# Hongyang-Du/VideoGPA

Measured on AMD Instinct MI355X. Metric: DPO preference-pair steps/sec, CogVideoX-5B 49f@480x720, higher is better.
Workload: dtype bf16; 1 GPU; BASELINE configs[1]: CogVideoX-5B T2V full (42 blocks, D=3072, 48x64 heads), 49f x 480x720 -> paired latents [1,2,13,16,60,90], S=17776 tokens, 42 blocks, LoRA r=64 on to_q/to_k/to_v/to_out.0, 1 pair/GPU/step, optimizer step every step; random-init weights; layers=42, pairs_per_gpu=1, parallelism=dp1

## Files before the change

### videogpa_amd/csrc/lora.hip

```cpp
#include "attn_w1.h"

#ifndef LORA_DOWN_DMA
#define LORA_DOWN_DMA 1
#endif
#ifndef LORA_DOWN_DMA_NCB
#define LORA_DOWN_DMA_NCB 2
#endif
#ifndef LORA_DOWN_NS
#define LORA_DOWN_NS 4
#endif
#ifndef LORA_GRAD_WGS
#define LORA_GRAD_WGS 768
#endif

#include <cstdlib>

__device__ __forceinline__ void tile_load_zfill(const bf16_t* base, int64_t ld, int64_t row0, int64_t nrows, int col0, int ncols,
                                                u32x4_t (&r)[2]) {
#pragma unroll
    for (int j = 0; j < 2; ++j) {
        const int c = threadIdx.x + 256 * j;
        const int64_t row = row0 + (c >> 3);
        const int col = col0 + (c & 7) * 8;
        u32x4_t z = {0u, 0u, 0u, 0u};
        r[j] = (row < nrows && col < ncols) ? *reinterpret_cast<const u32x4_t*>(base + row * ld + col) : z;
    }
}

template <int NCB>
__global__ __launch_bounds__(256) void lora_down_kernel(const bf16_t* __restrict__ X, int64_t ldx, const bf16_t* __restrict__ A,
                                                          bf16_t* __restrict__ T, int64_t ldt, int64_t M, int K, int R) {
    extern __shared__ __attribute__((aligned(16))) bf16_t smem[];
    constexpr int RP = 32 * NCB;
    constexpr int NACC = (NCB + 1) / 2;
    constexpr int BUF = (64 + RP) * PITCH;
    const int lane = threadIdx.x & 63, wave = threadIdx.x >> 6, hi = lane >> 5;
    const int rb = wave & 1, cg = wave >> 1;
    const int64_t row0 = (int64_t)blockIdx.x * 64;

    f32x16_t acc[NACC];
#pragma unroll
    for (int a = 0; a < NACC; ++a)
#pragma unroll
        for (int i = 0; i < 16; ++i) acc[a][i] = 0.f;

    u32x4_t xr[2], ar[NCB];
    auto load = [&](int k0) {
        tile_load_zfill(X, ldx, row0, M, k0, K, xr);
#pragma unroll
        for (int j = 0; j < NCB; ++j) {
            const int c = threadIdx.x + 256 * j;
            const int row = c >> 3;
            u32x4_t z = {0u, 0u, 0u, 0u};
            ar[j] = (row < R) ? *reinterpret_cast<const u32x4_t*>(A + (int64_t)row * K + k0 + (c & 7) * 8) : z;
        }
    };
    auto store = [&](int buf) {
        bf16_t* xl = smem + buf * BUF;
        bf16_t* al = xl + 64 * PITCH;
        tile_store(xl, xr);
#pragma unroll
        for (int j = 0; j < NCB; ++j) {
            const int c = threadIdx.x + 256 * j;
            *reinterpret_cast<u32x4_t*>(al + (c >> 3) * PITCH + (c & 7) * 8) = ar[j];
        }
    };
    const int nk = K / 64;
    load(0);
    store(0);
    __syncthreads();
    for (int t = 0; t < nk; ++t) {
        const bf16_t* xl = smem + (t & 1) * BUF;
        const bf16_t* al = xl + 64 * PITCH;
        if (t + 1 < nk) load((t + 1) * 64);
#pragma unroll
        for (int ks = 0; ks < 4; ++ks) {
            const bf16x8_t xf = frag_row(xl, rb * 32, ks, lane);
#pragma unroll
            for (int a = 0; a < NACC; ++a) {
                const int cb = cg + 2 * a;
                if (cb < NCB) acc[a] = mfma32(frag_row(al, cb * 32, ks, lane), xf, acc[a]);
            }
        }
        if (t + 1 < nk) store((t + 1) & 1);
        __syncthreads();
    }
    const int64_t m = row0 + rb * 32 + (lane & 31);
    if (m < M) {
#pragma unroll
        for (int a = 0; a < NACC; ++a) {
            const int cb = cg + 2 * a;
            if (cb < NCB) {
#pragma unroll
                for (int g = 0; g < 4; ++g) {
                    const int n = cb * 32 + 8 * g + 4 * hi;
                    if (n + 3 < R || n < R) {
                        if (n + 3 < R) {
                            u32x2_t w;
                            w[0] = pack_bf16x2(acc[a][4 * g], acc[a][4 * g + 1]);
                            w[1] = pack_bf16x2(acc[a][4 * g + 2], acc[a][4 * g + 3]);
                            *reinterpret_cast<u32x2_t*>(T + m * ldt + n) = w;
                        } else {
                            for (int i = 0; i < 4; ++i)
                                if (n + i < R) T[m * ldt + n + i] = f32_to_bf16(acc[a][4 * g + i]);
                        }
                    }
                }
            }
        }
    }
}

template <int N>
__device__ __forceinline__ void lora_wait_vm() { asm volatile("s_waitcnt vmcnt(%0) lgkmcnt(0)" ::"n"(N) : "memory"); }

template <int NCB, int NS>
__global__ __launch_bounds__(256) void lora_down_dma_kernel(const bf16_t* __restrict__ X, int64_t ldx, const bf16_t* __restrict__ A, bf16_t* __restrict__ T,
                                                              int64_t ldt, int64_t M, int K, int R) {
    constexpr int RP = 32 * NCB;
    constexpr int NACC = (NCB + 1) / 2;
    constexpr int STAGE = 8192 + RP * 128;
    constexpr int PW = 2 + NCB;
    __shared__ __attribute__((aligned(1024))) uint8_t lds[NS * STAGE];
    const int lane = threadIdx.x & 63, hi = lane >> 5;
    const int wave = __builtin_amdgcn_readfirstlane((int)threadIdx.x >> 6);
    const int rb = wave & 1, cg = wave >> 1;
    const int64_t row0 = (int64_t)blockIdx.x * 64;
    const int64_t rows = (M - row0) < 64 ? (M - row0) : 64;

    const W1Rsrc xrs = w1_rsrc(X + row0 * ldx, (uint32_t)(((rows - 1) * ldx + K) * 2));
    const W1Rsrc ars = w1_rsrc(A, (uint32_t)((int64_t)R * K * 2));
    uint32_t xo[2], ao[NCB];
#pragma unroll
    for (int i = 0; i < 2; ++i) {
        const uint32_t row = 8u * (uint32_t)(wave * 2 + i) + (uint32_t)(lane >> 3);
        xo[i] = (uint32_t)((row * (uint64_t)ldx + (((uint32_t)(lane & 7) ^ w1_swz(row)) * 8u)) * 2u);
    }
#pragma unroll
    for (int i = 0; i < NCB; ++i) {
        const uint32_t row = 8u * (uint32_t)(wave * NCB + i) + (uint32_t)(lane >> 3);
        ao[i] = (row * (uint32_t)K + (((uint32_t)(lane & 7) ^ w1_swz(row)) * 8u)) * 2u;
    }
    const uint32_t lds0 = (uint32_t)(uintptr_t)(__attribute__((address_space(3))) uint8_t*)lds;
    const uint32_t xdst = __builtin_amdgcn_readfirstlane(lds0 + (uint32_t)wave * 2048u);
    const uint32_t adst = __builtin_amdgcn_readfirstlane(lds0 + 8192u + (uint32_t)wave * (uint32_t)NCB * 1024u);
    auto issue = [&](int slot) {
        const uint32_t so = (uint32_t)slot * (uint32_t)STAGE;
#pragma unroll
        for (int i = 0; i < 2; ++i) { w1_dma(xdst + so + 1024u * i, xrs, xo[i], 0u); xo[i] += 128u; }
#pragma unroll
        for (int i = 0; i < NCB; ++i) { w1_dma(adst + so + 1024u * i, ars, ao[i], 0u); ao[i] += 128u; }
    };
    f32x16_t acc[NACC];
#pragma unroll
    for (int a = 0; a < NACC; ++a)
#pragma unroll
        for (int i = 0; i < 16; ++i) acc[a][i] = 0.f;
    const W1Lane la = w1_lane_offsets(lane);
    const int nk = K / 64;
#pragma unroll
    for (int t = 0; t < NS - 1; ++t) issue(t);
    for (int t = 0; t < nk; ++t) {
        lora_wait_vm<PW * (NS - 2)>();
        __syncthreads();
        issue((t + NS - 1) % NS);
        const uint32_t xb = (uint32_t)(t % NS) * (uint32_t)STAGE, ab = xb + 8192u;
#pragma unroll
        for (int ks = 0; ks < 4; ++ks) {
            const bf16x8_t xf = w1_frag_row(lds, xb, la, rb, ks);
#pragma unroll
            for (int a = 0; a < NACC; ++a) {
                const int cb = cg + 2 * a;
                if (cb < NCB) acc[a] = mfma32(w1_frag_row(lds, ab, la, cb, ks), xf, acc[a]);
            }
        }
    }
    lora_wait_vm<0>();
    const int64_t m = row0 + rb * 32 + (lane & 31);
    if (m < M) {
#pragma unroll
        for (int a = 0; a < NACC; ++a) {
            const int cb = cg + 2 * a;
            if (cb < NCB) {
#pragma unroll
                for (int g = 0; g < 4; ++g) {
                    const int n = cb * 32 + 8 * g + 4 * hi;
                    if (n + 3 < R) {
                        u32x2_t w;
                        w[0] = pack_bf16x2(acc[a][4 * g], acc[a][4 * g + 1]);
                        w[1] = pack_bf16x2(acc[a][4 * g + 2], acc[a][4 * g + 3]);
                        *reinterpret_cast<u32x2_t*>(T + m * ldt + n) = w;
                    } else {
                        for (int i = 0; i < 4; ++i)
                            if (n + i < R) T[m * ldt + n + i] = f32_to_bf16(acc[a][4 * g + i]);
                    }
                }
            }
        }
    }
}

#ifndef UP_COLS
#define UP_COLS 128
#endif
#define UP_PITCH (UP_COLS + 4)
template <int KS>
__global__ __launch_bounds__(256) void lora_up_add_kernel(bf16_t* __restrict__ Y, int64_t ldy, const bf16_t* __restrict__ T, int64_t ldt,
                                                            const bf16_t* __restrict__ Bw, int64_t ldb, float s, int64_t M, int N,
                                                            int accumulate) {
    __shared__ __attribute__((aligned(16))) float tile[64 * UP_PITCH];
    const int lane = threadIdx.x & 63, wave = threadIdx.x >> 6, hi = lane >> 5;
    const int64_t m0 = (int64_t)blockIdx.x * 64;
    const int n0 = blockIdx.y * UP_COLS;
    const int rb = wave & 1, cg = wave >> 1;
    int64_t mr = m0 + rb * 32 + (lane & 31);
    mr = mr < M ? mr : M - 1;
    bf16x8_t tf[KS];
#pragma unroll
    for (int ks = 0; ks < KS; ++ks) tf[ks] = *reinterpret_cast<const bf16x8_t*>(T + mr * ldt + ks * 16 + hi * 8);
#pragma unroll
    for (int cbi = 0; cbi < UP_COLS / 64; ++cbi) {
        const int nl = cg * (UP_COLS / 2) + cbi * 32;
        int nrow = n0 + nl + (lane & 31);
        nrow = nrow < N ? nrow : N - 1;
        f32x16_t acc;
#pragma unroll
        for (int i = 0; i < 16; ++i) acc[i] = 0.f;
        const bf16_t* bp = Bw + (int64_t)nrow * ldb + hi * 8;
#pragma unroll
        for (int ks = 0; ks < KS; ++ks) acc = mfma32(*reinterpret_cast<const bf16x8_t*>(bp + ks * 16), tf[ks], acc);
        float* tp = tile + (rb * 32 + (lane & 31)) * UP_PITCH + nl + 4 * hi;
#pragma unroll
        for (int g = 0; g < 4; ++g) {
            f32x4_t v = {s * acc[4 * g], s * acc[4 * g + 1], s * acc[4 * g + 2], s * acc[4 * g + 3]};
            *reinterpret_cast<f32x4_t*>(tp + 8 * g) = v;
        }
    }
    __syncthreads();
#pragma unroll
    for (int j = 0; j < UP_COLS / 32; ++j) {
        const int c = threadIdx.x + 256 * j;
        const int row = c / (UP_COLS / 8), col = (c % (UP_COLS / 8)) * 8;
        const int64_t m = m0 + row;
        if (m < M && n0 + col < N) {
            const float* tp = tile + row * UP_PITCH + col;
            const f32x4_t a0 = *reinterpret_cast<const f32x4_t*>(tp), a1 = *reinterpret_cast<const f32x4_t*>(tp + 4);
            float o[8] = {a0[0], a0[1], a0[2], a0[3], a1[0], a1[1], a1[2], a1[3]};
            bf16_t* yp = Y + m * ldy + n0 + col;
            if (accumulate) {
                float y[8];
                unpack8(*reinterpret_cast<const u32x4_t*>(yp), y);
#pragma unroll
                for (int i = 0; i < 8; ++i) o[i] += y[i];
            }
            *reinterpret_cast<u32x4_t*>(yp) = pack8(o);
        }
    }
}

__global__ __launch_bounds__(256) void lora_grad_kernel(const bf16_t* __restrict__ U, int64_t ldu, const bf16_t* __restrict__ V, int64_t ldv,
                                                          float* __restrict__ G, int64_t ldg, float s, int64_t M, int P, int Q,
                                                          int64_t rows_per_split, int n_qt, float* __restrict__ part) {
    __shared__ __attribute__((aligned(16))) bf16_t lds[4 * TILE_ELEMS];
    const int lane = threadIdx.x & 63, wave = threadIdx.x >> 6, hi = lane >> 5;
    const int pb = wave & 1, qb = wave >> 1;
    const int p0 = (blockIdx.x / n_qt) * 64, q0 = (blockIdx.x % n_qt) * 64;
    const int64_t mbeg = (int64_t)blockIdx.y * rows_per_split;
    int64_t mend = mbeg + rows_per_split;
    mend = mend < M ? mend : M;
    if (mbeg >= mend) return;
    f32x16_t acc;
#pragma unroll
    for (int i = 0; i < 16; ++i) acc[i] = 0.f;
    u32x4_t ur[2], vr[2];
    const int nt = (int)((mend - mbeg + 63) / 64);
    tile_load_zfill(U, ldu, mbeg, mend, p0, P, ur);
    tile_load_zfill(V, ldv, mbeg, mend, q0, Q, vr);
    tile_store(lds, ur);
    tile_store(lds + 2 * TILE_ELEMS, vr);
    __syncthreads();
    for (int t = 0; t < nt; ++t) {
        const bf16_t* ul = lds + (t & 1) * TILE_ELEMS;
        const bf16_t* vl = lds + (2 + (t & 1)) * TILE_ELEMS;
        if (t + 1 < nt) {
            tile_load_zfill(U, ldu, mbeg + (int64_t)(t + 1) * 64, mend, p0, P, ur);
            tile_load_zfill(V, ldv, mbeg + (int64_t)(t + 1) * 64, mend, q0, Q, vr);
        }
#pragma unroll
        for (int kc = 0; kc < 4; ++kc) acc = mfma32(frag_tr(ul, 16 * kc, pb * 32, lane), frag_tr(vl, 16 * kc, qb * 32, lane), acc);
        if (t + 1 < nt) {
            tile_store(lds + ((t + 1) & 1) * TILE_ELEMS, ur);
            tile_store(lds + (2 + ((t + 1) & 1)) * TILE_ELEMS, vr);
        }
        __syncthreads();
    }
    const int q = q0 + qb * 32 + (lane & 31);
    if (q < Q) {
        float* slab = part ? part + (int64_t)blockIdx.y * P * Q : nullptr;
#pragma unroll
        for (int r = 0; r < 16; ++r) {
            const int p = p0 + pb * 32 + acc_row(r, hi);
            if (p < P) {
                if (slab) slab[(int64_t)p * Q + q] = acc[r];
                else atomicAdd(&G[(int64_t)p * ldg + q], s * acc[r]);
            }
        }
    }
}

__global__ __launch_bounds__(256) void lora_grad_merge_kernel(const float* __restrict__ part, int nsplit, float* __restrict__ G, int64_t ldg, float s,
                                                                int P, int Q) {
    const int64_t i = (int64_t)blockIdx.x * 256 + threadIdx.x;
    if (i >= (int64_t)P * Q) return;
    float a = 0.f;
    for (int c = 0; c < nsplit; ++c) a += part[(int64_t)c * P * Q + i];
    G[(i / Q) * ldg + (i % Q)] = s * a;
}

__global__ __launch_bounds__(256) void lora_ext_refresh_kernel(const float* __restrict__ A, const float* __restrict__ B, float s, int r, int K, int Dn,
                                                                 bf16_t* __restrict__ a_cat, bf16_t* __restrict__ wt_tail, int64_t ld_wt,
                                                                 bf16_t* __restrict__ w_tail, int64_t ld_w, bf16_t* __restrict__ sbt) {
    const int64_t idx = (int64_t)blockIdx.x * 256 + threadIdx.x;
    const int64_t na = (int64_t)r * K;
    if (idx < na) {
        const int rr = (int)(idx / K), kk = (int)(idx % K);
        const bf16_t a = f32_to_bf16(A[idx]);
        a_cat[idx] = a;
        wt_tail[(int64_t)kk * ld_wt + rr] = a;
    } else if (idx < na + (int64_t)Dn * r) {
        const int64_t e = idx - na;
        const int n = (int)(e / r), rr = (int)(e % r);
        const bf16_t v = f32_to_bf16(bf16_to_f32(f32_to_bf16(B[e])) * s);
        w_tail[(int64_t)n * ld_w + rr] = v;
        sbt[(int64_t)rr * Dn + n] = v;
    }
}

static inline bool a16(const void* p) { return ((uintptr_t)p & 15) == 0; }
static inline bool a8(const void* p) { return ((uintptr_t)p & 7) == 0; }

extern "C" {

int32_t vgpa_lora_down(const void* X, int64_t ldx, const void* A, void* T, int64_t ldt, int64_t M, int64_t K, int64_t R, hipStream_t stream) {
    if (!X || !A || !T || M <= 0 || K <= 0 || K % 64 != 0 || R <= 0 || R > 256 || ldx % 8 || ldt % 8 || ldx < K || ldt < R || !a16(X) || !a16(A) || !a8(T))
        return VGPA_ERR_INVALID;
    if (M > ((int64_t)1 << 31) * 32) return VGPA_ERR_INVALID;
    const int ncb = (int)((R + 31) / 32);
    const dim3 grid((unsigned)((M + 63) / 64));
    constexpr bool dma_off = LORA_DOWN_DMA == 0;
    constexpr int dma_max_ncb = LORA_DOWN_DMA_NCB;
    if (!dma_off && ncb <= dma_max_ncb && (uint64_t)64 * (uint64_t)ldx * 2 + (uint64_t)K * 2 + 1024 < (1ull << 32) && ((uint64_t)R + 8) * (uint64_t)K * 2 + 1024 < (1ull << 32)) {
#define LDD(N, S) VGPA_LAUNCH((lora_down_dma_kernel<N, S>), grid, dim3(256), 0, stream, (const bf16_t*)X, ldx, (const bf16_t*)A, (bf16_t*)T, ldt, M, (int)K, (int)R)
        constexpr int ns = LORA_DOWN_NS;
        switch (ncb * 10 + ns) {
            case 14: LDD(1, 4); break; case 24: LDD(2, 4); break;
            case 13: LDD(1, 3); break; case 23: LDD(2, 3); break;
            case 63: LDD(6, 3); break; case 64: LDD(6, 4); break;
            default: return VGPA_ERR_INVALID;
        }
#undef LDD
        VGPA_CHECK_LAUNCH();
        return VGPA_OK;
    }
    const size_t shmem = (size_t)2 * (64 + 32 * ncb) * PITCH * sizeof(bf16_t);
#define LD(N)                                                                                                                      \
    if (hipFuncSetAttribute((const void*)lora_down_kernel<N>, hipFuncAttributeMaxDynamicSharedMemorySize, (int)shmem) != hipSuccess) \
        return VGPA_ERR_LAUNCH;                                                                                                    \
    VGPA_LAUNCH((lora_down_kernel<N>), grid, dim3(256), shmem, stream, (const bf16_t*)X, ldx, (const bf16_t*)A, (bf16_t*)T, ldt, M, (int)K, (int)R)
    switch (ncb) {
        case 1: LD(1); break; case 2: LD(2); break; case 3: LD(3); break; case 4: LD(4); break;
        case 5: LD(5); break; case 6: LD(6); break; case 7: LD(7); break; case 8: LD(8); break;
        default: return VGPA_ERR_INVALID;
    }
#undef LD
    VGPA_CHECK_LAUNCH();
    return VGPA_OK;
}

int32_t vgpa_lora_up_add(void* Y, int64_t ldy, const void* T, int64_t ldt, const void* Bw, int64_t ldb, float s, int64_t M, int64_t N,
                         int64_t rp, int32_t accumulate, hipStream_t stream) {
    if (!Y || !T || !Bw || M <= 0 || N <= 0 || N % 8 != 0 || ldy % 8 || ldt % 8 || ldb % 8 || !a16(T) || !a16(Bw) || !a16(Y))
        return VGPA_ERR_INVALID;
    if (ldy < N || ldt < rp || ldb < rp) return VGPA_ERR_INVALID;
    const dim3 grid((unsigned)((M + 63) / 64), (unsigned)((N + UP_COLS - 1) / UP_COLS));
#define UP(KS) VGPA_LAUNCH((lora_up_add_kernel<KS>), grid, dim3(256), 0, stream, (bf16_t*)Y, ldy, (const bf16_t*)T, ldt, (const bf16_t*)Bw, ldb, s, M, (int)N, (int)accumulate)
    switch (rp) {
        case 16: UP(1); break; case 32: UP(2); break; case 48: UP(3); break; case 64: UP(4); break;
        case 96: UP(6); break; case 128: UP(8); break; case 192: UP(12); break;
        default: return VGPA_ERR_INVALID;
    }
#undef UP
    VGPA_CHECK_LAUNCH();
    return VGPA_OK;
}

static void lora_grad_plan(int64_t M, int64_t P, int64_t Q, int* n_pt, int* n_qt, int64_t* rows, int64_t* splits) {
    *n_pt = (int)((P + 63) / 64);
    *n_qt = (int)((Q + 63) / 64);
    constexpr int64_t target = LORA_GRAD_WGS;
    int64_t sp = target / ((int64_t)*n_pt * *n_qt);
    if (sp < 1) sp = 1;
    const int64_t max_splits = (M + 255) / 256;
    if (sp > max_splits) sp = max_splits;
    int64_t r = (M + sp - 1) / sp;
    r = (r + 63) / 64 * 64;
    *rows = r;
    *splits = (M + r - 1) / r;
}

size_t vgpa_lora_grad_workspace_bytes(int64_t M, int64_t P, int64_t Q) {
    if (M <= 0 || P <= 0 || Q <= 0) return 0;
    int n_pt, n_qt;
    int64_t rows, splits;
    lora_grad_plan(M, P, Q, &n_pt, &n_qt, &rows, &splits);
    return (size_t)splits * (size_t)P * (size_t)Q * sizeof(float);
}
int32_t vgpa_lora_grad_ws(const void* U, int64_t ldu, const void* V, int64_t ldv, float* G, int64_t ldg, float s, int64_t M, int64_t P,
                          int64_t Q, void* workspace, size_t ws_bytes, hipStream_t stream) {
    if (!U || !V || !G || !workspace || M <= 0 || P <= 0 || Q <= 0 || P % 8 || Q % 8 || ldu % 8 || ldv % 8 || !a16(U) || !a16(V) || !a16(workspace))
        return VGPA_ERR_INVALID;
    if (ldu < P || ldv < Q || ldg < Q || ((uintptr_t)G & 3)) return VGPA_ERR_INVALID;
    int n_pt, n_qt;
    int64_t rows, splits;
    lora_grad_plan(M, P, Q, &n_pt, &n_qt, &rows, &splits);
    if (ws_bytes < (size_t)splits * (size_t)P * (size_t)Q * sizeof(float)) return VGPA_ERR_WORKSPACE;
    VGPA_LAUNCH(lora_grad_kernel, dim3((unsigned)(n_pt * n_qt), (unsigned)splits), dim3(256), 0, stream, (const bf16_t*)U, ldu, (const bf16_t*)V, ldv,
                G, ldg, s, M, (int)P, (int)Q, rows, n_qt, (float*)workspace);
    VGPA_CHECK_LAUNCH();
    VGPA_LAUNCH(lora_grad_merge_kernel, dim3((unsigned)((P * Q + 255) / 256)), dim3(256), 0, stream, (const float*)workspace, (int)splits, G, ldg, s,
                (int)P, (int)Q);
    VGPA_CHECK_LAUNCH();
    return VGPA_OK;
}

int32_t vgpa_lora_ext_refresh(const float* A, const float* B, float s, int64_t r, int64_t K, int64_t Dn, void* a_cat, void* wt_tail, int64_t ld_wt, void* w_tail,
                              int64_t ld_w, void* sbt, hipStream_t stream) {
    if (!A || !B || !a_cat || !wt_tail || !w_tail || !sbt || r <= 0 || K <= 0 || Dn <= 0 || ld_wt < r || ld_w < r) return VGPA_ERR_INVALID;
    const int64_t total = r * K + Dn * r;
    if (total >= ((int64_t)1 << 31)) return VGPA_ERR_INVALID;
    VGPA_LAUNCH(lora_ext_refresh_kernel, dim3((unsigned)((total + 255) / 256)), dim3(256), 0, stream, A, B, s, (int)r, (int)K, (int)Dn, (bf16_t*)a_cat, (bf16_t*)wt_tail,
                ld_wt, (bf16_t*)w_tail, ld_w, (bf16_t*)sbt);
    VGPA_CHECK_LAUNCH();
    return VGPA_OK;
}

}
```

Before: 0.4490 pair-steps/s.

## Add multi-stage DMA ring streaming kernel for LoRA down projection

Adds a new LoRA down-projection kernel that keeps separate multi-buffered LDS rings for X and A tiles, issues async buffer DMAs interleaved with MFMA steps, and sizes the rows per workgroup from CU slot count and LDS budget. For ranks of 2 or 6 column blocks (r=64 in this workload), dispatch now goes to this streaming path with default ring depths (RB=5, NX=3, NA=3) ahead of the older DMA kernel. The aim is deeper prefetch, so the memory-bound X read better overlaps compute and occupancy is balanced across the grid. In exchange it uses large LDS rings, which limits concurrent workgroups, and adds tricky vmcnt bookkeeping.

```diff
diff --git a/videogpa_amd/csrc/lora.hip b/videogpa_amd/csrc/lora.hip
--- a/videogpa_amd/csrc/lora.hip
+++ b/videogpa_amd/csrc/lora.hip
@@ -11,6 +11,12 @@
 #endif
 #ifndef LORA_GRAD_WGS
 #define LORA_GRAD_WGS 768
+#endif
+#ifndef LORA_DOWN_STREAM2
+#define LORA_DOWN_STREAM2 533
+#endif
+#ifndef LORA_DOWN_STREAM6
+#define LORA_DOWN_STREAM6 533
 #endif
 
 #include <cstdlib>
@@ -193,6 +199,124 @@
                     } else {
                         for (int i = 0; i < 4; ++i)
                             if (n + i < R) T[m * ldt + n + i] = f32_to_bf16(acc[a][4 * g + i]);
+                    }
+                }
+            }
+        }
+    }
+}
+
+template <int NCB, int RB, int NX, int NA>
+__global__ __launch_bounds__(256) void lora_down_stream_kernel(const bf16_t* __restrict__ X, int64_t ldx, const bf16_t* __restrict__ A, bf16_t* __restrict__ T,
+                                                                 int64_t ldt, int64_t M, int K, int R, int rows_wg) {
+    constexpr int XB = RB * 4096, AB = NCB * 4096;
+    constexpr int NRA = (RB + 1) / 2, NCA = (NCB + 1) / 2;
+    constexpr int FLY = (NX > NA ? RB : 0) + (NA - 2) * (RB + NCB);
+    static_assert(NA >= 2 && NA <= NX && FLY <= 63, "ring depths against the vmcnt field");
+    static_assert(NCB % 2 == 0, "two waves share the column blocks evenly: the main loop has no branch");
+    __shared__ __attribute__((aligned(1024))) uint8_t ring[NX * XB + NA * AB];
+    const int lane = threadIdx.x & 63, hi = lane >> 5;
+    const int wave = __builtin_amdgcn_readfirstlane((int)threadIdx.x >> 6);
+    const int rg = wave & 1, cg = wave >> 1;
+    const int64_t row0 = (int64_t)blockIdx.x * rows_wg;
+    if (row0 >= M) return;
+    const int rows = (int)((M - row0) < rows_wg ? (M - row0) : rows_wg);
+
+    const W1Rsrc xrs = w1_rsrc(X + row0 * ldx, (uint32_t)(((int64_t)(rows - 1) * ldx + K) * 2));
+    const W1Rsrc ars = w1_rsrc(A, (uint32_t)((int64_t)R * K * 2));
+    uint32_t xo[RB], ao[NCB];
+#pragma unroll
+    for (int i = 0; i < RB; ++i) {
+        const uint32_t row = 8u * (uint32_t)(wave * RB + i) + (uint32_t)(lane >> 3);
+        xo[i] = (uint32_t)((row * (uint64_t)ldx + (((uint32_t)(lane & 7) ^ w1_swz(row)) * 8u)) * 2u);
+    }
+#pragma unroll
+    for (int i = 0; i < NCB; ++i) {
+        const uint32_t row = 8u * (uint32_t)(wave * NCB + i) + (uint32_t)(lane >> 3);
+        ao[i] = (row * (uint32_t)K + (((uint32_t)(lane & 7) ^ w1_swz(row)) * 8u)) * 2u;
+    }
+    const uint32_t lds0 = (uint32_t)(uintptr_t)(__attribute__((address_space(3))) uint8_t*)ring;
+    const uint32_t xdst = __builtin_amdgcn_readfirstlane(lds0 + (uint32_t)wave * (uint32_t)RB * 1024u);
+    const uint32_t adst = __builtin_amdgcn_readfirstlane(lds0 + (uint32_t)(NX * XB) + (uint32_t)wave * (uint32_t)NCB * 1024u);
+    int xin = 0, ain = 0;
+    auto ask = [&](int p) {
+        if (p < NCB) w1_dma(adst + (uint32_t)ain * (uint32_t)AB + 1024u * p, ars, ao[p], 0u), ao[p] += 128u;
+        else w1_dma(xdst + (uint32_t)xin * (uint32_t)XB + 1024u * (p - NCB), xrs, xo[p - NCB], 0u), xo[p - NCB] += 128u;
+    };
+    auto asked = [&](bool with_a) {
+        if (with_a) ain = ain + 1 == NA ? 0 : ain + 1;
+        xin = xin + 1 == NX ? 0 : xin + 1;
+    };
+    f32x16_t acc[NRA][NCA];
+#pragma unroll
+    for (int a = 0; a < NRA; ++a)
+#pragma unroll
+        for (int c = 0; c < NCA; ++c)
+#pragma unroll
+            for (int i = 0; i < 16; ++i) acc[a][c][i] = 0.f;
+    int rbs[NRA];
+#pragma unroll
+    for (int a = 0; a < NRA; ++a) rbs[a] = rg + 2 * a < RB ? rg + 2 * a : RB - 1;
+    const W1Lane la = w1_lane_offsets(lane);
+    const int nk = K / 64;
+#pragma unroll
+    for (int i = -(NX - 1); i < 0; ++i) {
+#pragma unroll
+        for (int p = (i + NA - 1 >= 0 ? 0 : NCB); p < NCB + RB; ++p) ask(p);
+        asked(i + NA - 1 >= 0);
+    }
+    int xout = 0, aout = 0;
+    constexpr int NG = 4 * NRA;
+    for (int t = 0; t < nk; ++t) {
+        lora_wait_vm<FLY>();
+        __syncthreads();
+        const uint32_t xb = (uint32_t)xout * (uint32_t)XB, ab = (uint32_t)(NX * XB) + (uint32_t)aout * (uint32_t)AB;
+        xout = xout + 1 == NX ? 0 : xout + 1;
+        aout = aout + 1 == NA ? 0 : aout + 1;
+        bf16x8_t af[2][NCA], xf[2][NRA];
+        auto frags = [&](int ks) {
+#pragma unroll
+            for (int c = 0; c < NCA; ++c) af[ks & 1][c] = w1_frag_row(ring, ab, la, cg + 2 * c, ks);
+#pragma unroll
+            for (int a = 0; a < NRA; ++a) xf[ks & 1][a] = w1_frag_row(ring, xb, la, rbs[a], ks);
+        };
+        frags(0);
+#pragma unroll
+        for (int ks = 0; ks < 4; ++ks) {
+            if (ks < 3) frags(ks + 1);
+#pragma unroll
+            for (int a = 0; a < NRA; ++a) {
+#pragma unroll
+                for (int c = 0; c < NCA; ++c) acc[a][c] = mfma32(af[ks & 1][c], xf[ks & 1][a], acc[a][c]);
+                constexpr int P = NCB + RB;
+                const int g = ks * NRA + a;
+#pragma unroll
+                for (int p = g * P / NG; p < (g + 1) * P / NG; ++p) ask(p);
+            }
+        }
+        asked(true);
+    }
+    lora_wait_vm<0>();
+#pragma unroll
+    for (int a = 0; a < NRA; ++a) {
+        const int ml = (rg + 2 * a) * 32 + (lane & 31);
+        if (rg + 2 * a >= RB || ml >= rows) continue;
+        const int64_t m = row0 + ml;
+#pragma unroll
+        for (int c = 0; c < NCA; ++c) {
+            const int cb = cg + 2 * c;
+            if (cb < NCB) {
+#pragma unroll
+                for (int g = 0; g < 4; ++g) {
+                    const int n = cb * 32 + 8 * g + 4 * hi;
+                    if (n + 3 < R) {
+                        u32x2_t w;
+                        w[0] = pack_bf16x2(acc[a][c][4 * g], acc[a][c][4 * g + 1]);
+                        w[1] = pack_bf16x2(acc[a][c][4 * g + 2], acc[a][c][4 * g + 3]);
+                        *reinterpret_cast<u32x2_t*>(T + m * ldt + n) = w;
+                    } else {
+                        for (int i = 0; i < 4; ++i)
+                            if (n + i < R) T[m * ldt + n + i] = f32_to_bf16(acc[a][c][4 * g + i]);
                     }
                 }
             }
@@ -339,6 +463,23 @@
 static inline bool a16(const void* p) { return ((uintptr_t)p & 15) == 0; }
 static inline bool a8(const void* p) { return ((uintptr_t)p & 7) == 0; }
 
+static inline bool lora_stream_addressable(int ncb, int rb, int nx, int64_t ldx, int64_t K) {
+    return (uint64_t)(32 * rb) * (uint64_t)ldx * 2 + (uint64_t)K * 2 + (uint64_t)nx * 128 + 1024 < (1ull << 32) &&
+           ((uint64_t)(32 * ncb) + 8) * (uint64_t)K * 2 + (uint64_t)nx * 128 + 1024 < (1ull << 32);
+}
+template <int NCB, int RB, int NX, int NA>
+static int32_t lora_down_stream(const void* X, int64_t ldx, const void* A, void* T, int64_t ldt, int64_t M, int64_t K, int64_t R, hipStream_t stream) {
+    constexpr int ring = (NX * RB + NA * NCB) * 4096;
+    static_assert(ring <= 160 * 1024, "the rings must fit a CU's LDS");
+    const int64_t slots = (int64_t)(wg_slots() / 2) * (160 * 1024 / ring);
+    int64_t rows = (M + slots - 1) / slots;
+    rows = rows < 32 ? 32 : (rows > 32 * RB ? 32 * RB : rows);
+    VGPA_LAUNCH((lora_down_stream_kernel<NCB, RB, NX, NA>), dim3((unsigned)((M + rows - 1) / rows)), dim3(256), 0, stream, (const bf16_t*)X, ldx, (const bf16_t*)A,
+                (bf16_t*)T, ldt, M, (int)K, (int)R, (int)rows);
+    VGPA_CHECK_LAUNCH();
+    return VGPA_OK;
+}
+
 extern "C" {
 
 int32_t vgpa_lora_down(const void* X, int64_t ldx, const void* A, void* T, int64_t ldt, int64_t M, int64_t K, int64_t R, hipStream_t stream) {
@@ -346,6 +487,14 @@
         return VGPA_ERR_INVALID;
     if (M > ((int64_t)1 << 31) * 32) return VGPA_ERR_INVALID;
     const int ncb = (int)((R + 31) / 32);
+#define LDS_ARM(N, V_)                                                         \
+    {                                                                          \
+        constexpr int V = V_ ? V_ : 533;  \
+        if (ncb == N && V_ && lora_stream_addressable(N, V / 100, V / 10 % 10, ldx, K)) return lora_down_stream<N, V / 100, V / 10 % 10, V % 10>(X, ldx, A, T, ldt, M, K, R, stream); \
+    }
+    LDS_ARM(2, LORA_DOWN_STREAM2);
+    LDS_ARM(6, LORA_DOWN_STREAM6);
+#undef LDS_ARM
     const dim3 grid((unsigned)((M + 63) / 64));
     constexpr bool dma_off = LORA_DOWN_DMA == 0;
     constexpr int dma_max_ncb = LORA_DOWN_DMA_NCB;
```

New measurement: 0.4488 pair-steps/s. Within noise of the previous version (-0.1%).
